# marlbenchmark/off-policy

Hardware: NVIDIA H100
Metric: learner grad-steps/sec (higher is better)
Workload: dtype f32

## Files before the change

### off-policy_b200/csrc/agent_bwd.cu

```cuda
#include "mx_internal.h"
#include "mx_kernels.h"
#include "mx_tile.cuh"
#include "mx_mma.cuh"

static inline size_t qhead_bwd_smem(int A) { return (size_t)(A * MX_H * 9 + 8 * 32 + 2 * 8 * MX_H + 2 * MX_H) * sizeof(float); }

__global__ void __launch_bounds__(256) k_qhead_bwd(QHeadBwdArgs a) {
  MX_DYN_SMEM(smem);
  const int tid = threadIdx.x, lane = tid & 31, warp = tid >> 5;
  const int A = a.A, AW = A * MX_H;
  float* wq_s = smem;
  float* dw_w = wq_s + AW;
  float* db_w = dw_w + 8 * AW;
  float* dg_w = db_w + 8 * 32;
  float* dbt_w = dg_w + 8 * MX_H;
  float* lg_s = dbt_w + 8 * MX_H;
  float* lb_s = lg_s + MX_H;
  for (int i = tid; i < AW; i += blockDim.x) wq_s[i] = a.theta[a.wq + i];
  for (int i = tid; i < 8 * AW + 8 * 32; i += blockDim.x) dw_w[i] = 0.f;
  for (int i = tid; i < MX_H; i += blockDim.x) { lg_s[i] = a.theta[a.lno_g + i]; lb_s[i] = a.theta[a.lno_b + i]; }
  MX_PDL_WAIT();
  __syncthreads();
  const int wglobal = blockIdx.x * (blockDim.x >> 5) + warp;
  const int wtotal = gridDim.x * (blockDim.x >> 5);
// ... 247 lines not shown
        if (rok[r]) mx_cp16z(pf_dst + ((t & (RING - 1)) * ROWS + r) * (6 * MX_H), first ? (pf_h0[r] ? pf_h0[r] : a.hall) : pf_src[r], (first && !pf_h0[r]) ? 0 : 16);
        pf_src[r] -= pf_stride;
      }
    }
    mx_cp_commit();
  };
  if (ROWS > 1) {
    for (int idx = tid; idx < RING * ROWS * 6 * MX_H; idx += BWD2_THREADS) (&ops_s[0][0][0][0])[idx] = 0.f;
    __syncthreads();
  }
#pragma unroll
  for (int d = 0; d < PF; ++d) prefetch(t_first - d);
  mx_cp_wait<PF - 1>();
  __syncthreads();

  auto step = [&](const int t, const int cur) {
    prefetch(t - PF);
    float cz[ROWS];
#pragma unroll
    for (int r = 0; r < ROWS; ++r) {
      const float* o = &ops_s[t & (RING - 1)][r][0][0];
      const float rg = o[ku], zg = o[MX_H + ku], ng = o[2 * MX_H + ku], hn = o[3 * MX_H + ku], hp = o[4 * MX_H + ku];
      const float dh = o[5 * MX_H + ku] + carry[r];
      const float d_n = dh * (1.f - zg) * (1.f - ng * ng);
      const float d_z = dh * (hp - ng) * zg * (1.f - zg);
      const float d_r = d_n * hn * rg * (1.f - rg);
      dgh_s[cur][r][(half ? 2 * MX_H : 0) + ku] = half ? d_n * rg : d_r;
      if (!half) dgh_s[cur][r][MX_H + ku] = d_z;
      if (rok[r]) {
        dgp[r][half ? 2 * MX_H : 0] = half ? d_n : d_r;
        if (!half) dgp[r][MX_H] = d_z;
      }
      dgp[r] -= dg_stride;
      cz[r] = dh * zg;
    }
    mx_cp_wait<PF - 1>();
    __syncthreads();
#pragma unroll
    for (int r = 0; r < ROWS; ++r) {
      float2 a0 = make_float2(0.f, 0.f), a1 = a0, b0 = a0, b1 = a0;
#pragma unroll
      for (int m = 0; m < 12; ++m) {
        const float4 d = mx_ld4(&dgh_s[cur][r][16 * m + 4 * s]);
        const float2 lo = make_float2(d.x, d.y), hi = make_float2(d.z, d.w);
        a0 = mx_ffma2(w0[2 * m], lo, a0); b0 = mx_ffma2(w1[2 * m], lo, b0);
        a1 = mx_ffma2(w0[2 * m + 1], hi, a1); b1 = mx_ffma2(w1[2 * m + 1], hi, b1);
      }
      a0 = mx_fadd2(a0, a1); b0 = mx_fadd2(b0, b1);
      float p0 = a0.x + a0.y, p1 = b0.x + b0.y;
      p0 += __shfl_xor_sync(0xffffffffu, p0, 1); p1 += __shfl_xor_sync(0xffffffffu, p1, 1);
      p0 += __shfl_xor_sync(0xffffffffu, p0, 2); p1 += __shfl_xor_sync(0xffffffffu, p1, 2);
      carry[r] = cz[r] + ((s & 1) ? p1 : p0);
    }
  };
  int t = t_first;
  for (; t >= 1; t -= 2) { step(t, 0); step(t - 1, 1); }
  if (t == 0) step(0, 0);
  mx_cp_wait<0>();
}

struct FrontBwdSmem {
  int ldi, ld64, ldg;
  int o_dgi, o_dgn, o_x, o_hp, o_u, o_da, o_x0, o_xh0, o_dx0, o_wc, o_col, o_stat, o_lnp, total;
};
static FrontBwdSmem front_bwd_smem(int in_dim, int TM, bool gru_ext = false) {
  FrontBwdSmem s;
  const int I64 = mx_round_up(in_dim, 64);
  s.ldi = mx_ld(I64); s.ld64 = mx_ld(64); s.ldg = mx_ld(MX_G);
  int o = 0;
  s.o_dgi = o; o += TM * s.ldg;
  s.o_dgn = o; o += gru_ext ? 0 : TM * s.ld64;
  s.o_x = o; o += TM * s.ld64;
  s.o_hp = o; o += gru_ext ? 0 : TM * s.ld64;
  s.o_u = o; o += TM * s.ld64;
  s.o_da = o; o += TM * s.ld64;
  s.o_x0 = o; o += TM * s.ldi;
  s.o_xh0 = o; o += TM * s.ldi;
  s.o_dx0 = o; o += TM * s.ldi;
  s.o_wc = o; o += 64 * s.ld64;
  s.o_col = o; o += 2 * I64 + 4 * 64;
  s.o_stat = o; o += 3 * TM * 2;
  s.o_lnp = o; o += 4 * 64;
  s.total = o;
  return s;
}

template <int RM>
MX_DEVINL void ln64_bwd_relu(bool act_tanh, float (&v)[RM][4], const float* u_s, int ld, const float* stat , const float* gamma_s,
                             float (&dg)[4], float (&db)[4]) {
  const int tx = threadIdx.x & 15, ty = threadIdx.x >> 4;
#pragma unroll
  for (int i = 0; i < RM; ++i) {
    const int r = ty * RM + i;
    const float mean = stat[2 * r], rstd = stat[2 * r + 1];
    const float4 u4 = mx_ld4(u_s + r * ld + 4 * tx);
    const float uu[4] = {u4.x, u4.y, u4.z, u4.w};
    float xh[4], dx[4], s1 = 0.f, s2 = 0.f;
#pragma unroll
    for (int j = 0; j < 4; ++j) {
      xh[j] = (uu[j] - mean) * rstd;
      dg[j] = fmaf(v[i][j], xh[j], dg[j]);
      db[j] += v[i][j];
      dx[j] = v[i][j] * gamma_s[4 * tx + j];
      s1 += dx[j]; s2 += dx[j] * xh[j];
    }
    s1 = mx_row16_sum(s1) * (1.f / 64.f);
    s2 = mx_row16_sum(s2) * (1.f / 64.f);
#pragma unroll
    for (int j = 0; j < 4; ++j) {
      const float du = rstd * (dx[j] - s1 - xh[j] * s2);
      v[i][j] = act_tanh ? du * (1.f - uu[j] * uu[j]) : (uu[j] > 0.f ? du : 0.f);
    }
  }
}

template <int RM, bool MMA>
__global__ void __launch_bounds__(MX_TILE_THREADS) k_front_bwd(FrontBwdArgs a, FrontBwdSmem sm) {
  constexpr int TM = 16 * RM;
  MX_DYN_SMEM(smem);
  const MxNetLayout L = a.L;
  const float* __restrict__ th = a.theta;
  const int I = L.in_dim, I64 = mx_round_up(I, 64);
  float* dgi_s = smem + sm.o_dgi; float* dgn_s = smem + sm.o_dgn; float* x_s = smem + sm.o_x; float* hp_s = smem + sm.o_hp;
  float* u_s = smem + sm.o_u; float* da_s = smem + sm.o_da; float* x0_s = smem + sm.o_x0; float* xh0_s = smem + sm.o_xh0;
  float* Wc = smem + sm.o_wc;
  float* col0g = smem + sm.o_col; float* col0b = col0g + I64;
  float* col1g = col0b + I64; float* col1b = col1g + 64;
  float* col2g = col1b + 64; float* col2b = col2g + 64;
  float* st0_s = smem + sm.o_stat; float* st1_s = st0_s + 2 * TM; float* st2_s = st1_s + 2 * TM;
  float* ln1g_s = smem + sm.o_lnp; float* ln1b_s = ln1g_s + 64; float* ln2g_s = ln1b_s + 64; float* ln2b_s = ln2g_s + 64;
  const int tid = threadIdx.x, tx = tid & 15, ty = tid >> 4;
  const int ntiles = (a.M + TM - 1) / TM;
  const int T1 = a.T1 > 0 ? a.T1 : a.T + 1, N = a.N;
  const bool ldx_vec = (a.ldx & 3) == 0;
  const bool wg = !a.skip_wgrad;
  const bool wgemm = wg && !a.wgrad_external;
  const bool gru_here = !a.gru_wgrad_ext;
  float* dx0_s = smem + sm.o_dx0;
  float* gp = a.gpart + (size_t)blockIdx.x * a.P;
  for (int i = tid; i < 2 * I64 + 4 * 64; i += MX_TILE_THREADS) col0g[i] = 0.f;
  if (tid < 64) { ln1g_s[tid] = th[L.ln1_g + tid]; ln1b_s[tid] = th[L.ln1_b + tid]; ln2g_s[tid] = th[L.ln2_g + tid]; ln2b_s[tid] = th[L.ln2_b + tid]; }
  float dg1[4] = {0.f, 0.f, 0.f, 0.f}, db1[4] = {0.f, 0.f, 0.f, 0.f}, dg2[4] = {0.f, 0.f, 0.f, 0.f}, db2[4] = {0.f, 0.f, 0.f, 0.f};
  int iter = 0;
  MX_PDL_WAIT();
  for (int tile = blockIdx.x; tile < ntiles; tile += gridDim.x, ++iter) {
    const int m0 = tile * TM;
    const bool accum = iter > 0;
    __syncthreads();
    mx_stage_rows(dgi_s, sm.ldg, a.dgi, MX_G, m0, a.M, TM, MX_G);
    if (!gru_here) {}
    else if (!a.no_gru) mx_stage_rows(x_s, sm.ld64, a.gates, MX_G, m0, a.M, TM, MX_H);
    else for (int i = tid; i < TM * sm.ld64; i += MX_TILE_THREADS) x_s[i] = 0.f;
    mx_stage_rows(u_s, sm.ld64, a.u2, MX_H, m0, a.M, TM, MX_H);
    for (int r = tid >> 4; gru_here && r < TM; r += MX_TILE_THREADS / 16) {
      const int m = m0 + r;
      const bool has = !a.no_gru && m < a.M && ((m / N) % T1) > 0;
      float* d = hp_s + r * sm.ld64 + 4 * tx;
      if (has) mx_cp16(d, a.hall + (size_t)(m - N) * MX_H + 4 * tx);
      else if (m < a.M && a.h0) mx_cp16(d, a.h0 + (size_t)m * MX_H + 4 * tx);
      else mx_st4(d, make_float4(0.f, 0.f, 0.f, 0.f));
    }
    if (ldx_vec) mx_stage_rows(x0_s, sm.ldi, a.X, a.ldx, m0, a.M, TM, mx_round_up(I, 4));
    mx_cp_commit();
    for (int i = tid; i < 3 * TM * 2; i += MX_TILE_THREADS) {
      const int which = i / (2 * TM), rr = (i % (2 * TM)) >> 1, comp = i & 1;
      const int m = m0 + rr;
      const float* src = which == 0 ? a.st0 : (which == 1 ? a.st1 : a.st2);
      st0_s[i] = (m < a.M && (which > 0 || a.feature_norm)) ? src[2 * (size_t)m + comp] : 0.f;
    }
    mx_cp_wait<0>();
    __syncthreads();
    for (int idx = tid; gru_here && idx < TM * MX_H; idx += MX_TILE_THREADS) {
      const int r = idx >> 6, c = idx & 63;
      const int o = r * sm.ld64 + c;
      dgn_s[o] = dgi_s[r * sm.ldg + 2 * MX_H + c] * x_s[o];
      x_s[o] = (m0 + r < a.M) ? (u_s[o] - st2_s[2 * r]) * st2_s[2 * r + 1] * ln2g_s[c] + ln2b_s[c] : 0.f;
    }
    __syncthreads();
    if (wgemm && gru_here) {
      for (int nb = 0; nb < 3; ++nb) {
        if (MMA) mx_mma_wgrad_block(dgi_s + nb * 64, sm.ldg, x_s, sm.ld64, TM, gp + L.wih, MX_G, MX_H, nb * 64, 0, accum);
        else mx_wgrad_block(dgi_s + nb * 64, sm.ldg, x_s, sm.ld64, TM, gp + L.wih, MX_G, MX_H, nb * 64, 0, accum);
        if (a.no_gru) continue;
        const float* dgh = nb < 2 ? dgi_s + nb * 64 : dgn_s;
        const int ldd = nb < 2 ? sm.ldg : sm.ld64;
        if (MMA) mx_mma_wgrad_block(dgh, ldd, hp_s, sm.ld64, TM, gp + L.whh + nb * 64 * MX_H, 64, MX_H, 0, 0, accum);
        else mx_wgrad_block(dgh, ldd, hp_s, sm.ld64, TM, gp + L.whh + nb * 64 * MX_H, 64, MX_H, 0, 0, accum);
      }
      mx_colsum(dgi_s, sm.ldg, TM, MX_G, gp + L.bih, accum);
      if (!a.no_gru) {
        mx_colsum(dgi_s, sm.ldg, TM, 2 * MX_H, gp + L.bhh, accum);
        mx_colsum(dgn_s, sm.ld64, TM, MX_H, gp + L.bhh + 2 * MX_H, accum);
      }
    }
    float v[RM][4];
#pragma unroll
    for (int i = 0; i < RM; ++i)
#pragma unroll
      for (int jx = 0; jx < 4; ++jx) v[i][jx] = 0.f;
    if (MMA) {
      float cfr[RM][4];
#pragma unroll
      for (int i = 0; i < RM; ++i)
#pragma unroll
        for (int jx = 0; jx < 4; ++jx) cfr[i][jx] = 0.f;
      for (int nc = 0; nc < 3; ++nc) {
        __syncthreads();
        mx_stage_weight(Wc, sm.ld64, th + L.wih, MX_G, MX_H, MX_H, nc * 64, 0, 64);
        __syncthreads();
        mx_mma_dgrad_acc<RM>(cfr, dgi_s + nc * 64, sm.ldg, Wc, sm.ld64);
      }
      mx_mma_store<RM>(cfr, da_s, sm.ld64);
      __syncthreads();
#pragma unroll
      for (int i = 0; i < RM; ++i) {
        const float4 q = mx_ld4(da_s + (ty * RM + i) * sm.ld64 + 4 * tx);
        v[i][0] = q.x; v[i][1] = q.y; v[i][2] = q.z; v[i][3] = q.w;
      }
    } else
    for (int nc = 0; nc < 3; ++nc) {
      __syncthreads();
      mx_stage_weight(Wc, sm.ld64, th + L.wih, MX_G, MX_H, MX_H, nc * 64, 0, 64);
      __syncthreads();
      mx_mm_nn<RM>(dgi_s + nc * 64, sm.ldg, Wc, sm.ld64, v);
    }
    ln64_bwd_relu<RM>(a.act_tanh != 0, v, u_s, sm.ld64, st2_s, ln2g_s, dg2, db2);
    __syncthreads();
#pragma unroll
    for (int i = 0; i < RM; ++i) mx_st4(da_s + (ty * RM + i) * sm.ld64 + 4 * tx, make_float4(v[i][0], v[i][1], v[i][2], v[i][3]));
    if (a.wgrad_external) {
#pragma unroll
      for (int i = 0; i < RM; ++i) {
        const int m = m0 + ty * RM + i;
        if (m < a.M) mx_st4(a.da2_out + (size_t)m * MX_H + 4 * tx, make_float4(v[i][0], v[i][1], v[i][2], v[i][3]));
      }
    }
    mx_stage_rows(u_s, sm.ld64, a.u1, MX_H, m0, a.M, TM, MX_H);
    mx_cp_commit();
    mx_cp_wait<0>();
    __syncthreads();
    for (int idx = tid; idx < TM * MX_H; idx += MX_TILE_THREADS) {
      const int r = idx >> 6, c = idx & 63;
      const int o = r * sm.ld64 + c;
      x_s[o] = (m0 + r < a.M) ? (u_s[o] - st1_s[2 * r]) * st1_s[2 * r + 1] * ln1g_s[c] + ln1b_s[c] : 0.f;
    }
    __syncthreads();
    if (wgemm) {
      if (MMA) mx_mma_wgrad_block(da_s, sm.ld64, x_s, sm.ld64, TM, gp + L.w2, MX_H, MX_H, 0, 0, accum);
      else mx_wgrad_block(da_s, sm.ld64, x_s, sm.ld64, TM, gp + L.w2, MX_H, MX_H, 0, 0, accum);
      mx_colsum(da_s, sm.ld64, TM, MX_H, gp + L.b2, accum);
    }
    mx_stage_weight(Wc, sm.ld64, th + L.w2, MX_H, MX_H, MX_H, 0, 0, 64);
    __syncthreads();
#pragma unroll
    for (int i = 0; i < RM; ++i)
#pragma unroll
      for (int jx = 0; jx < 4; ++jx) v[i][jx] = 0.f;
    if (MMA) {
      float cfr[RM][4];
#pragma unroll
      for (int i = 0; i < RM; ++i)
#pragma unroll
        for (int jx = 0; jx < 4; ++jx) cfr[i][jx] = 0.f;
      mx_mma_dgrad_acc<RM>(cfr, da_s, sm.ld64, Wc, sm.ld64);
      mx_mma_store<RM>(cfr, x_s, sm.ld64);
      __syncthreads();
#pragma unroll
      for (int i = 0; i < RM; ++i) {
        const float4 q = mx_ld4(x_s + (ty * RM + i) * sm.ld64 + 4 * tx);
        v[i][0] = q.x; v[i][1] = q.y; v[i][2] = q.z; v[i][3] = q.w;
      }
    } else
    mx_mm_nn<RM>(da_s, sm.ld64, Wc, sm.ld64, v);
    ln64_bwd_relu<RM>(a.act_tanh != 0, v, u_s, sm.ld64, st1_s, ln1g_s, dg1, db1);
    __syncthreads();
#pragma unroll
    for (int i = 0; i < RM; ++i) mx_st4(da_s + (ty * RM + i) * sm.ld64 + 4 * tx, make_float4(v[i][0], v[i][1], v[i][2], v[i][3]));
    if (a.wgrad_external) {
#pragma unroll
      for (int i = 0; i < RM; ++i) {
        const int m = m0 + ty * RM + i;
        if (m < a.M) mx_st4(a.da1_out + (size_t)m * MX_H + 4 * tx, make_float4(v[i][0], v[i][1], v[i][2], v[i][3]));
      }
    }
    for (int idx = tid; idx < TM * I64; idx += MX_TILE_THREADS) {
      const int r = idx / I64, c = idx - r * I64, m = m0 + r;
      float xh = 0.f, x0 = 0.f;
      if (m < a.M && c < I) {
        const float x = ldx_vec ? x0_s[r * sm.ldi + c] : a.X[(size_t)m * a.ldx + c];
        if (a.feature_norm) {
          xh = (x - st0_s[2 * r]) * st0_s[2 * r + 1];
          x0 = xh * th[L.fn_g + c] + th[L.fn_b + c];
        } else x0 = x;
      }
      x0_s[r * sm.ldi + c] = x0; xh0_s[r * sm.ldi + c] = xh;
    }
    __syncthreads();
    if (wgemm) {
      for (int kb = 0; kb * 64 < I; ++kb) {
        if (MMA) mx_mma_wgrad_block(da_s, sm.ld64, x0_s + kb * 64, sm.ldi, TM, gp + L.w1, MX_H, I, 0, kb * 64, accum);
        else mx_wgrad_block(da_s, sm.ld64, x0_s + kb * 64, sm.ldi, TM, gp + L.w1, MX_H, I, 0, kb * 64, accum);
      }
      mx_colsum(da_s, sm.ld64, TM, MX_H, gp + L.b1, accum);
    }
    if (a.feature_norm || a.dX) {
      for (int kb = 0; kb * 64 < I; ++kb) {
        __syncthreads();
        mx_stage_weight(Wc, sm.ld64, th + L.w1, MX_H, I, I, 0, kb * 64, 64);
        __syncthreads();
#pragma unroll
        for (int i = 0; i < RM; ++i)
#pragma unroll
          for (int jx = 0; jx < 4; ++jx) v[i][jx] = 0.f;
        if (MMA) {
          float cfr[RM][4];
#pragma unroll
          for (int i = 0; i < RM; ++i)
#pragma unroll
            for (int jx = 0; jx < 4; ++jx) cfr[i][jx] = 0.f;
          mx_mma_dgrad_acc<RM>(cfr, da_s, sm.ld64, Wc, sm.ld64);
          mx_mma_store<RM>(cfr, dx0_s + kb * 64, sm.ldi);
          __syncthreads();
#pragma unroll
          for (int i = 0; i < RM; ++i) {
            const float4 q = mx_ld4(dx0_s + (ty * RM + i) * sm.ldi + kb * 64 + 4 * tx);
            v[i][0] = q.x; v[i][1] = q.y; v[i][2] = q.z; v[i][3] = q.w;
          }
        } else
        mx_mm_nn<RM>(da_s, sm.ld64, Wc, sm.ld64, v);
        float cg[4] = {0.f, 0.f, 0.f, 0.f}, cb[4] = {0.f, 0.f, 0.f, 0.f};
#pragma unroll
        for (int jx = 0; jx < 4; ++jx) {
          const int c = kb * 64 + 4 * tx + jx;
          if (c < I) {
            float sg = 0.f, sb = 0.f;
#pragma unroll
            for (int i = 0; i < RM; ++i) {
              sg = fmaf(v[i][jx], xh0_s[(ty * RM + i) * sm.ldi + c], sg); sb += v[i][jx];
              if (a.dX) dx0_s[(ty * RM + i) * sm.ldi + c] = v[i][jx];
            }
            cg[jx] = sg; cb[jx] = sb;
          }
        }
        if (wg && a.feature_norm) {
          for (int g = 0; g < MX_TILE_THREADS / 16; ++g) {
            if (ty == g) {
#pragma unroll
              for (int jx = 0; jx < 4; ++jx) {
                const int c = kb * 64 + 4 * tx + jx;
                if (c < I) { col0g[c] += cg[jx]; col0b[c] += cb[jx]; }
              }
            }
            __syncthreads();
          }
        }
      }
      if (a.dX) {
        __syncthreads();
        const int lane = tid & 31, warp = tid >> 5;
        for (int r = warp; r < TM; r += MX_TILE_THREADS / 32) {
          const int m = m0 + r;
          if (m >= a.M) continue;
          float s1 = 0.f, s2 = 0.f;
          for (int c = lane; c < I; c += 32) {
            const float dxh = dx0_s[r * sm.ldi + c] * (a.feature_norm ? th[L.fn_g + c] : 1.f);
            s1 += dxh; s2 += dxh * xh0_s[r * sm.ldi + c];
          }
          s1 = mx_warp_sum(s1) / (float)I; s2 = mx_warp_sum(s2) / (float)I;
          const float rstd = st0_s[2 * r + 1];
          for (int c = lane; c < I; c += 32) {
            const float d0 = dx0_s[r * sm.ldi + c];
            a.dX[(size_t)m * a.ldx + c] = a.feature_norm ? rstd * (d0 * th[L.fn_g + c] - s1 - xh0_s[r * sm.ldi + c] * s2) : d0;
          }
        }
      }
    }
  }
  for (int g = 0; g < MX_TILE_THREADS / 16; ++g) {
    if (ty == g) {
#pragma unroll
      for (int jx = 0; jx < 4; ++jx) {
        const int c = 4 * tx + jx;
        col1g[c] += dg1[jx]; col1b[c] += db1[jx];
        col2g[c] += dg2[jx]; col2b[c] += db2[jx];
      }
    }
    __syncthreads();
  }
  if (wg) {
    for (int c = tid; c < MX_H; c += MX_TILE_THREADS) {
      gp[L.ln2_g + c] = col2g[c]; gp[L.ln2_b + c] = col2b[c];
      gp[L.ln1_g + c] = col1g[c]; gp[L.ln1_b + c] = col1b[c];
    }
    for (int c = tid; c < I; c += MX_TILE_THREADS) { gp[L.fn_g + c] = col0g[c]; gp[L.fn_b + c] = col0b[c]; }
  }
}


struct GruWgradSmem { int ld64, ldg, o_dgi, o_dgn, o_x, o_hp, o_stat, o_lnp, total; };
static GruWgradSmem gru_wgrad_smem(int TM) {
  GruWgradSmem s;
  s.ld64 = mx_ld(64); s.ldg = mx_ld(MX_G);
  int o = 0;
  s.o_dgi = o; o += TM * s.ldg;
  s.o_dgn = o; o += TM * s.ld64;
  s.o_x = o; o += TM * s.ld64;
  s.o_hp = o; o += TM * s.ld64;
  s.o_stat = o; o += 2 * TM;
  s.o_lnp = o; o += 2 * 64;
  s.total = o;
  return s;
}

template <int RM>
__global__ void __launch_bounds__(MX_TILE_THREADS, 2) k_gru_wgrad(FrontBwdArgs a, GruWgradSmem sm) {
  constexpr int TM = 16 * RM;
  MX_DYN_SMEM(smem);
  const MxNetLayout L = a.L;
  const float* __restrict__ th = a.theta;
  float* dgi_s = smem + sm.o_dgi; float* dgn_s = smem + sm.o_dgn; float* x_s = smem + sm.o_x; float* hp_s = smem + sm.o_hp;
  float* st2_s = smem + sm.o_stat; float* ln2g_s = smem + sm.o_lnp; float* ln2b_s = ln2g_s + 64;
  const int tid = threadIdx.x, tx = tid & 15;
  const int tk = tid & 7, tn = tid >> 3;
  const int ntiles = (a.M + TM - 1) / TM;
  const int T1 = a.T1 > 0 ? a.T1 : a.T + 1, N = a.N;
  float* gp = a.gpart + (size_t)blockIdx.x * a.P;
  if (tid < 64) { ln2g_s[tid] = th[L.ln2_g + tid]; ln2b_s[tid] = th[L.ln2_b + tid]; }
  int iter = 0;
  MX_PDL_WAIT();
  for (int tile = blockIdx.x; tile < ntiles; tile += gridDim.x, ++iter) {
    const int m0 = tile * TM;
    __syncthreads();
    mx_stage_rows(dgi_s, sm.ldg, a.dgi, MX_G, m0, a.M, TM, MX_G);
    mx_stage_rows(dgn_s, sm.ld64, a.gates, MX_G, m0, a.M, TM, MX_H);
    mx_stage_rows(x_s, sm.ld64, a.u2, MX_H, m0, a.M, TM, MX_H);
    for (int r = tid >> 4; r < TM; r += MX_TILE_THREADS / 16) {
      const int m = m0 + r;
      const bool has = m < a.M && ((m / N) % T1) > 0;
// ... 68 lines not shown
  const int cap = mx_num_sms();
  if (grid > cap) grid = cap;
  if (grid < 1) grid = 1;
  const size_t smem = qhead_bwd_smem(a.A);
#if !MX_EMU
  static size_t configured = 0;
  if (smem > 48 * 1024 && smem > configured) {
    if (cudaFuncSetAttribute(k_qhead_bwd, cudaFuncAttributeMaxDynamicSharedMemorySize, (int)smem) != cudaSuccess) { mx_set_error("qhead_bwd: smem %zu too large", smem); return 1; }
    configured = smem;
  }
#endif
  MX_LAUNCH_PDL(k_qhead_bwd, dim3(grid), dim3(256), smem, s, a);
  MX_COUNT();
  MX_MARK("k_qhead_bwd", s);
  *nparts_used = grid;
  return MX_CHECK_LAUNCH("qhead_bwd");
}

__global__ void __launch_bounds__(256) k_mlp_dgi(const float* __restrict__ dq_taken, const int32_t* __restrict__ act_idx, int ld_tn,
                                                 float* __restrict__ dgi, int B, int N) {
  const long long total = (long long)B * 2 * N * MX_G;
  MX_PDL_WAIT();
  for (long long i = (long long)blockIdx.x * blockDim.x + threadIdx.x; i < total; i += (long long)gridDim.x * blockDim.x) {
    const int c = (int)(i % MX_G);
    const long long m = i / MX_G;
    const int n = (int)(m % N);
    const long long bt = m / N;
    const int t = (int)(bt & 1);
    const long long b = bt >> 1;
    float v = 0.f;
    if (t == 0 && c == act_idx[b * ld_tn + n]) v = dq_taken[b * N + n];
    dgi[i] = v;
  }
}
int mx_launch_mlp_dgi(const float* dq_taken, const int32_t* act_idx, int ld_tn, float* dgi, int B, int N, cudaStream_t s) {
  const long long total = (long long)B * 2 * N * MX_G;
  int grid = (int)((total + 255) / 256);
  const int cap = mx_num_sms() * 8;
  if (grid > cap) grid = cap;
  MX_LAUNCH_PDL(k_mlp_dgi, dim3(grid), dim3(256), 0, s, dq_taken, act_idx, ld_tn, dgi, B, N);
  MX_COUNT();
  MX_MARK("k_mlp_dgi", s);
  return MX_CHECK_LAUNCH("mlp_dgi");
}

int mx_launch_gru_bwd(const GruBwdArgs& a, cudaStream_t s) {
  const int sms = mx_num_sms();
  int rpc = 1;
  while (rpc < 4 && mx_ceil_div(a.R, rpc) > 2 * sms) rpc *= 2;
  if (g_mx_gru_bwd_rpc == 1 || g_mx_gru_bwd_rpc == 2 || g_mx_gru_bwd_rpc == 4) rpc = g_mx_gru_bwd_rpc;
  if (g_mx_gru_threads == 128 || (g_mx_gru_threads == 0 && g_mx_gru_bwd_rpc == 0 && a.T >= 8)) {
    const bool two = g_mx_gru_rows == 2 || (g_mx_gru_rows == 0 && a.R > 2 * mx_num_sms());
    if (two) MX_LAUNCH_PDL(k_gru_bwd2<2>, dim3((a.R + 1) / 2), dim3(BWD2_THREADS), 0, s, a);
    else MX_LAUNCH_PDL(k_gru_bwd2<1>, dim3(a.R), dim3(BWD2_THREADS), 0, s, a);
    MX_COUNT();
    MX_MARK("k_gru_bwd", s);
    return MX_CHECK_LAUNCH("gru_bwd2");
  }
  dim3 grid(mx_ceil_div(a.R, rpc));
  if (rpc == 1) MX_LAUNCH_PDL(k_gru_bwd<1>, grid, dim3(BWD_THREADS), 0, s, a);
  else if (rpc == 2) MX_LAUNCH_PDL(k_gru_bwd<2>, grid, dim3(BWD_THREADS), 0, s, a);
  else MX_LAUNCH_PDL(k_gru_bwd<4>, grid, dim3(BWD_THREADS), 0, s, a);
  MX_COUNT();
  MX_MARK("k_gru_bwd", s);
  return MX_CHECK_LAUNCH("gru_bwd");
}

static int front_bwd_pick_rm(int M, int in_dim, int sms, bool gru_ext) {
  int best = 2;
  double best_cost = 1e30;
  for (int rm = 2; rm <= 4; ++rm) {
    FrontBwdSmem sm = front_bwd_smem(in_dim, 16 * rm, gru_ext);
    if ((size_t)sm.total * sizeof(float) + 16 > 227 * 1024) continue;
    const int tiles = mx_ceil_div(M, 16 * rm);
    const double cost = (double)mx_ceil_div(tiles, sms) * (1.0 + rm);
    if (cost < best_cost - 1e-9) { best_cost = cost; best = rm; }
  }
  return best;
}

template <int RM, bool MMA>
static int front_bwd_launch(const FrontBwdArgs& a, int* nparts_used, cudaStream_t s) {
  const int TM = 16 * RM;
  FrontBwdSmem sm = front_bwd_smem(a.L.in_dim, TM, a.gru_wgrad_ext != 0);
  const size_t smem = (size_t)sm.total * sizeof(float) + 16;
  const int ntiles = mx_ceil_div(a.M, TM);
  int grid = mx_num_sms();
  if (grid > ntiles) grid = ntiles;
  auto kern = k_front_bwd<RM, MMA>;
#if !MX_EMU
  if (smem > 227 * 1024) { mx_set_error("front_bwd: %zu bytes of shared memory needed (obs_dim too large)", smem); return 1; }
  static size_t configured = 0;
  if (smem > configured) { cudaFuncSetAttribute(kern, cudaFuncAttributeMaxDynamicSharedMemorySize, (int)smem); configured = smem; }
#endif
  MX_LAUNCH_PDL(kern, dim3(grid), dim3(MX_TILE_THREADS), smem, s, a, sm);
  MX_COUNT();
  MX_MARK("k_front_bwd", s);
  *nparts_used = grid;
  return MX_CHECK_LAUNCH("front_bwd");
}

extern int g_mx_front_bwd_rm;
int g_mx_gru_wgrad_split = 1;
int g_mx_front_bwd_mma = 0;
bool mx_front_bwd_tc_usable(const FrontBwdArgs& a);
int mx_launch_front_bwd_tc(const FrontBwdArgs& a, int* nparts_used, cudaStream_t s);
// ... 47 lines not shown
```

### off-policy_b200/csrc/agent_fwd.cu

```cuda
#include "mx_internal.h"
#include "mx_kernels.h"
#include "mx_tile.cuh"

template <int RM>
__global__ void __launch_bounds__(MX_TILE_THREADS) k_front_fwd(FrontFwdArgs a) {
  constexpr int TM = 16 * RM;
  MX_DYN_SMEM(smem);
  const int net = blockIdx.y;
  const float* __restrict__ th = a.theta[net];
  const MxNetLayout L = a.L;
  const int I = L.in_dim, Ipad = (I + 3) & ~3;
  const int lda = mx_ld_dev(Ipad > MX_H ? Ipad : MX_H);
  const int ldw = lda;
  float* A_s = smem;
  float* Wc = A_s + TM * lda;
  const int tid = threadIdx.x, tx = tid & 15, ty = tid >> 4, lane = tid & 31, warp = tid >> 5;
  const bool live = (net == 0);
  const int ntiles = (a.M + TM - 1) / TM;
  MX_PDL_WAIT();

  for (int tile = blockIdx.x; tile < ntiles; tile += gridDim.x) {
    const int m0 = tile * TM;
    if (I <= 128) {
      constexpr int RW = TM / (MX_TILE_THREADS / 32);
// ... 265 lines not shown
  const bool on1 = q == 0 || live, on2 = live, on3 = live && q == 0;
  const size_t s1 = (size_t)N * ((q == 0) ? MX_H : MX_G), s2 = (size_t)N * MX_G, s3 = (size_t)N * MX_H;
  float* pf_dst = &gi_s[0][0][4 * (pf_on ? tid : 0)];
  const size_t pf_stride = (size_t)N * MX_G;
  auto prefetch = [&](int t) {
    if (pf_on && t < T1) {
#pragma unroll
      for (int r = 0; r < ROWS; ++r) {
        if (rok[r]) mx_cp16(pf_dst + ((t & (GRU_RING - 1)) * ROWS + r) * MX_G, pf_src[r]);
        pf_src[r] += pf_stride;
      }
    }
    mx_cp_commit();
  };
#pragma unroll
  for (int t = 0; t < GRU_PF; ++t) prefetch(t);
  mx_cp_wait<GRU_PF - 1>();
  __syncthreads();

  auto step = [&](const int t, const int cur) {
    const int nxt = cur ^ 1;
    prefetch(t + GRU_PF);
#pragma unroll
    for (int r = 0; r < ROWS; ++r) {
      const float* g = &gi_s[t & (GRU_RING - 1)][r][0];
      const float* hrow = &h_s[cur][r][0];
      float4 hv[8];
#pragma unroll
      for (int m = 0; m < 8; ++m) hv[m] = mx_ld4(hrow + 8 * m + 4 * q);
      const float gr = g[i] + br, gz = g[MX_H + i] + bz, gn = g[2 * MX_H + i], hp = hrow[i];
      float2 r0 = make_float2(0.f, 0.f), r1 = r0, z0 = r0, z1 = r0, n0 = r0, n1 = r0;
#pragma unroll
      for (int m = 0; m < 8; ++m) {
        const float2 lo = make_float2(hv[m].x, hv[m].y), hi = make_float2(hv[m].z, hv[m].w);
        r0 = mx_ffma2(wr[2 * m], lo, r0); n0 = mx_ffma2(wn[2 * m], lo, n0); z0 = mx_ffma2(wz[2 * m], lo, z0);
        r1 = mx_ffma2(wr[2 * m + 1], hi, r1); n1 = mx_ffma2(wn[2 * m + 1], hi, n1); z1 = mx_ffma2(wz[2 * m + 1], hi, z1);
      }
      r0 = mx_fadd2(r0, r1); n0 = mx_fadd2(n0, n1); z0 = mx_fadd2(z0, z1);
      float pr = r0.x + r0.y, pn = n0.x + n0.y, pz = z0.x + z0.y;
      pr += __shfl_xor_sync(0xffffffffu, pr, 1); pn += __shfl_xor_sync(0xffffffffu, pn, 1); pz += __shfl_xor_sync(0xffffffffu, pz, 1);
      const float rg = mx_sigmoid_fast(pr + gr);
      const float hn = pn + bn;
      const float ng = mx_tanh_fast(fmaf(rg, hn, gn));
      const float zg = mx_sigmoid_fast(pz + gz);
      const float hnew = fmaf(zg, hp - ng, ng);
      h_s[nxt][r][i] = hnew;
      if (rok[r]) {
        if (on1) *p1[r] = q == 0 ? hnew : zg;
        if (on2) *p2[r] = q == 0 ? rg : ng;
        if (on3) *p3[r] = hn;
      }
      p1[r] += s1; p2[r] += s2; p3[r] += s3;
    }
    mx_cp_wait<GRU_PF - 1>();
    __syncthreads();
  };
  int t = 0;
  for (; t + 1 < T1; t += 2) { step(t, 0); step(t + 1, 1); }
  if (t < T1) step(t, 0);
  mx_cp_wait<0>();
}

__global__ void __launch_bounds__(256) k_qhead(QHeadArgs a) {
  __shared__ float wq_s[2][32 * MX_H];
  __shared__ float bq_s[2][32];
  __shared__ float lg_s[2][MX_H], lb_s[2][MX_H];
  const int tid = threadIdx.x, lane = tid & 31;
  const int A = a.A;
  for (int net = 0; net < 2; ++net) {
    const float* th = a.theta[net];
    for (int i = tid; i < A * MX_H; i += blockDim.x) wq_s[net][i] = th[a.wq + i];
    for (int i = tid; i < A; i += blockDim.x) bq_s[net][i] = th[a.bq + i];
    for (int i = tid; i < MX_H; i += blockDim.x) { lg_s[net][i] = th[a.lno_g + i]; lb_s[net][i] = th[a.lno_b + i]; }
  }
  MX_PDL_WAIT();
  __syncthreads();
  const int wglobal = blockIdx.x * (blockDim.x >> 5) + (tid >> 5);
  const int wtotal = gridDim.x * (blockDim.x >> 5);
  const int T1 = a.T + 1, N = a.N;
  for (int m = wglobal; m < a.M; m += wtotal) {
    const int n = m % N;
    const int bt = m / N;
    const int t = bt % T1, b = bt / T1;
    float q_live_at_act = 0.f, tq_sel = 0.f;
    int greedy = 0;
    const float* hl = a.hall[0] + (size_t)m * MX_H;
    const float* ht = a.hall[1] + (size_t)m * MX_H;
    const float hl0 = hl[lane], hl1 = hl[lane + 32], ht0 = ht[lane], ht1 = ht[lane + 32];
    const int act = (t < a.T) ? a.act_idx[(size_t)b * a.ld_tn + (size_t)t * N + n] : 0;
    float av = 1.f;
    if (a.avail && lane < A) av = a.avail[(size_t)m * a.act_ld + lane];
    const unsigned avail_mask = __ballot_sync(0xffffffffu, av != 0.f);
    {
      const float mean = mx_warp_sum(hl0 + hl1) * (1.f / MX_H);
      const float d0 = hl0 - mean, d1 = hl1 - mean;
      const float rstd = rsqrtf(mx_warp_sum(d0 * d0 + d1 * d1) * (1.f / MX_H) + MX_LN_EPS);
      if (lane == 0) { a.sto[2 * (size_t)m] = mean; a.sto[2 * (size_t)m + 1] = rstd; }
      const float y0 = d0 * rstd * lg_s[0][lane] + lb_s[0][lane];
      const float y1 = d1 * rstd * lg_s[0][lane + 32] + lb_s[0][lane + 32];
      float best = 0.f;
      for (int k = 0; k < A; ++k) {
        float q = mx_warp_sum(y0 * wq_s[0][k * MX_H + lane] + y1 * wq_s[0][k * MX_H + lane + 32]) + bq_s[0][k];
        if (a.qall0 && lane == 0) a.qall0[(size_t)m * A + k] = q;
        if (k == act) q_live_at_act = q;
        const float qm = ((avail_mask >> k) & 1u) ? q : -1e10f;
        if (k == 0 || qm > best) { best = qm; greedy = k; }
// ... 79 lines not shown

int mx_launch_pack_prev_act(const float* obs, int obs_ld, const float* acts, int act_ld, float* X, int ldx, int B, int T, int N, int O, int A,
                            cudaStream_t s) {
  const long long total = (long long)B * (T + 1) * N * ldx;
  int grid = (int)((total + 255) / 256);
  const int cap = mx_num_sms() * 8;
  if (grid > cap) grid = cap;
  MX_LAUNCH_PDL(k_pack_prev_act, dim3(grid), dim3(256), 0, s, obs, obs_ld, acts, act_ld, X, ldx, B, T, N, O, A);
  MX_COUNT();
  MX_MARK("k_pack_prev_act", s);
  return MX_CHECK_LAUNCH("pack_prev_act");
}

size_t mx_front_fwd_smem(int in_dim, int RM) {
  const int Ipad = mx_round_up(in_dim, 4);
  const int lda = mx_ld(Ipad > MX_H ? Ipad : MX_H);
  return (size_t)(16 * RM + 64) * lda * sizeof(float);
}

extern int g_mx_front_tc;
int mx_launch_front_fwd_tc(const FrontFwdArgs& a, int nets, cudaStream_t s);
bool mx_front_tc_usable(int in_dim, bool have_image);

int mx_launch_front_fwd(const FrontFwdArgs& a, int nets, cudaStream_t s) {
  if (mx_front_tc_usable(a.L.in_dim, a.tc_img[0] != nullptr) && (a.ldx & 3) == 0) return mx_launch_front_fwd_tc(a, nets, s);
  const int RM = 2;
  const int ntiles = mx_ceil_div(a.M, 16 * RM);
  int gx = mx_num_sms() / nets;
  if (gx < 1) gx = 1;
  if (gx > ntiles) gx = ntiles;
  const size_t smem = mx_front_fwd_smem(a.L.in_dim, RM);
  auto kern = k_front_fwd<2>;
#if !MX_EMU
  static size_t configured = 0;
  if (smem > configured) {
    if (cudaFuncSetAttribute(kern, cudaFuncAttributeMaxDynamicSharedMemorySize, (int)smem) != cudaSuccess) { mx_set_error("front_fwd: smem %zu too large", smem); return 1; }
    configured = smem;
  }
#endif
  MX_LAUNCH_PDL(kern, dim3(gx, nets), dim3(MX_TILE_THREADS), smem, s, a);
  MX_COUNT();
  MX_MARK("k_front_fwd", s);
  return MX_CHECK_LAUNCH("front_fwd");
}

int mx_launch_gru_fwd(const GruFwdArgs& a, int nets, cudaStream_t s) {
  const int sms = mx_num_sms();
  int rpc = 1;
  while (rpc < 4 && mx_ceil_div(a.R, rpc) * nets > 2 * sms) rpc *= 2;
  if (g_mx_gru_fwd_rpc == 1 || g_mx_gru_fwd_rpc == 2 || g_mx_gru_fwd_rpc == 4) rpc = g_mx_gru_fwd_rpc;
  if (g_mx_gru_threads == 128 || (g_mx_gru_threads == 0 && g_mx_gru_fwd_rpc == 0 && a.T + 1 >= 8)) {
    const bool two = g_mx_gru_rows == 2 || (g_mx_gru_rows == 0 && (long long)a.R * nets > 2LL * mx_num_sms());
    if (two) MX_LAUNCH_PDL(k_gru_fwd2<2>, dim3((a.R + 1) / 2, nets), dim3(GRU2_THREADS), 0, s, a);
    else MX_LAUNCH_PDL(k_gru_fwd2<1>, dim3(a.R, nets), dim3(GRU2_THREADS), 0, s, a);
    MX_COUNT();
    MX_MARK("k_gru_fwd", s);
    return MX_CHECK_LAUNCH("gru_fwd2");
  }
  dim3 grid(mx_ceil_div(a.R, rpc), nets);
  if (rpc == 1) MX_LAUNCH_PDL(k_gru_fwd<1>, grid, dim3(GRU_THREADS), 0, s, a);
  else if (rpc == 2) MX_LAUNCH_PDL(k_gru_fwd<2>, grid, dim3(GRU_THREADS), 0, s, a);
  else MX_LAUNCH_PDL(k_gru_fwd<4>, grid, dim3(GRU_THREADS), 0, s, a);
  MX_COUNT();
  MX_MARK("k_gru_fwd", s);
  return MX_CHECK_LAUNCH("gru_fwd");
}

int mx_launch_qhead(const QHeadArgs& a, cudaStream_t s) {
  if (a.A > 32) { mx_set_error("qhead: act_dim %d > 32 unsupported", a.A); return 1; }
  int grid = mx_ceil_div(a.M, 8);
  const int cap = mx_num_sms() * 4;
  if (grid > cap) grid = cap;
  MX_LAUNCH_PDL(k_qhead, dim3(grid), dim3(256), 0, s, a);
  MX_COUNT();
  MX_MARK("k_qhead", s);
  return MX_CHECK_LAUNCH("qhead");
}
```

Baseline: 4731.

## Prefetch MLP weight chunks asynchronously and parallelize LN column reductions

Issues asynchronous cp.async staging of the first weight chunk for each dgrad GEMM (wih, w2, w1) earlier, so the copies overlap with the preceding elementwise work and the barriers around them drop away. It also replaces the serialized per-row-group accumulation loops (one __syncthreads per group) for the feature-norm and layernorm gamma/beta gradients with a shared-memory partial buffer followed by a parallel column reduction. The cost is reuse of dgi_s as scratch and more fragile ordering of async copies and barriers.

```diff
diff --git a/off-policy_b200/csrc/agent_bwd.cu b/off-policy_b200/csrc/agent_bwd.cu
--- a/off-policy_b200/csrc/agent_bwd.cu
+++ b/off-policy_b200/csrc/agent_bwd.cu
@@ -413,11 +413,13 @@
   if (tid < 64) { ln1g_s[tid] = th[L.ln1_g + tid]; ln1b_s[tid] = th[L.ln1_b + tid]; ln2g_s[tid] = th[L.ln2_g + tid]; ln2b_s[tid] = th[L.ln2_b + tid]; }
   float dg1[4] = {0.f, 0.f, 0.f, 0.f}, db1[4] = {0.f, 0.f, 0.f, 0.f}, dg2[4] = {0.f, 0.f, 0.f, 0.f}, db2[4] = {0.f, 0.f, 0.f, 0.f};
   int iter = 0;
+  mx_stage_weight(Wc, sm.ld64, th + L.wih, MX_G, MX_H, MX_H, 0, 0, 64, false);
   MX_PDL_WAIT();
   for (int tile = blockIdx.x; tile < ntiles; tile += gridDim.x, ++iter) {
     const int m0 = tile * TM;
     const bool accum = iter > 0;
     __syncthreads();
+    if (iter > 0) mx_stage_weight(Wc, sm.ld64, th + L.wih, MX_G, MX_H, MX_H, 0, 0, 64, false);
     mx_stage_rows(dgi_s, sm.ldg, a.dgi, MX_G, m0, a.M, TM, MX_G);
     if (!gru_here) {}
     else if (!a.no_gru) mx_stage_rows(x_s, sm.ld64, a.gates, MX_G, m0, a.M, TM, MX_H);
@@ -476,27 +478,32 @@
 #pragma unroll
         for (int jx = 0; jx < 4; ++jx) cfr[i][jx] = 0.f;
       for (int nc = 0; nc < 3; ++nc) {
+        if (nc > 0) {
+          __syncthreads();
+          mx_stage_weight(Wc, sm.ld64, th + L.wih, MX_G, MX_H, MX_H, nc * 64, 0, 64);
+          __syncthreads();
+        }
+        mx_mma_dgrad_acc<RM>(cfr, dgi_s + nc * 64, sm.ldg, Wc, sm.ld64);
+      }
+      mx_mma_store<RM>(cfr, da_s, sm.ld64);
+      __syncthreads();
+#pragma unroll
+      for (int i = 0; i < RM; ++i) {
+        const float4 q = mx_ld4(da_s + (ty * RM + i) * sm.ld64 + 4 * tx);
+        v[i][0] = q.x; v[i][1] = q.y; v[i][2] = q.z; v[i][3] = q.w;
+      }
+    } else
+    for (int nc = 0; nc < 3; ++nc) {
+      if (nc > 0) {
         __syncthreads();
         mx_stage_weight(Wc, sm.ld64, th + L.wih, MX_G, MX_H, MX_H, nc * 64, 0, 64);
         __syncthreads();
-        mx_mma_dgrad_acc<RM>(cfr, dgi_s + nc * 64, sm.ldg, Wc, sm.ld64);
-      }
-      mx_mma_store<RM>(cfr, da_s, sm.ld64);
-      __syncthreads();
-#pragma unroll
-      for (int i = 0; i < RM; ++i) {
-        const float4 q = mx_ld4(da_s + (ty * RM + i) * sm.ld64 + 4 * tx);
-        v[i][0] = q.x; v[i][1] = q.y; v[i][2] = q.z; v[i][3] = q.w;
-      }
-    } else
-    for (int nc = 0; nc < 3; ++nc) {
-      __syncthreads();
-      mx_stage_weight(Wc, sm.ld64, th + L.wih, MX_G, MX_H, MX_H, nc * 64, 0, 64);
-      __syncthreads();
+      }
       mx_mm_nn<RM>(dgi_s + nc * 64, sm.ldg, Wc, sm.ld64, v);
     }
     ln64_bwd_relu<RM>(a.act_tanh != 0, v, u_s, sm.ld64, st2_s, ln2g_s, dg2, db2);
     __syncthreads();
+    mx_stage_weight(Wc, sm.ld64, th + L.w2, MX_H, MX_H, MX_H, 0, 0, 64, false);
 #pragma unroll
     for (int i = 0; i < RM; ++i) mx_st4(da_s + (ty * RM + i) * sm.ld64 + 4 * tx, make_float4(v[i][0], v[i][1], v[i][2], v[i][3]));
     if (a.wgrad_external) {
@@ -521,7 +528,6 @@
       else mx_wgrad_block(da_s, sm.ld64, x_s, sm.ld64, TM, gp + L.w2, MX_H, MX_H, 0, 0, accum);
       mx_colsum(da_s, sm.ld64, TM, MX_H, gp + L.b2, accum);
     }
-    mx_stage_weight(Wc, sm.ld64, th + L.w2, MX_H, MX_H, MX_H, 0, 0, 64);
     __syncthreads();
 #pragma unroll
     for (int i = 0; i < RM; ++i)
@@ -545,6 +551,8 @@
     mx_mm_nn<RM>(da_s, sm.ld64, Wc, sm.ld64, v);
     ln64_bwd_relu<RM>(a.act_tanh != 0, v, u_s, sm.ld64, st1_s, ln1g_s, dg1, db1);
     __syncthreads();
+    const bool dx0_wanted = a.feature_norm || a.dX;
+    if (dx0_wanted) mx_stage_weight(Wc, sm.ld64, th + L.w1, MX_H, I, I, 0, 0, 64, false);
 #pragma unroll
     for (int i = 0; i < RM; ++i) mx_st4(da_s + (ty * RM + i) * sm.ld64 + 4 * tx, make_float4(v[i][0], v[i][1], v[i][2], v[i][3]));
     if (a.wgrad_external) {
@@ -574,10 +582,11 @@
       }
       mx_colsum(da_s, sm.ld64, TM, MX_H, gp + L.b1, accum);
     }
-    if (a.feature_norm || a.dX) {
+    if (dx0_wanted) {
       for (int kb = 0; kb * 64 < I; ++kb) {
         __syncthreads();
-        mx_stage_weight(Wc, sm.ld64, th + L.w1, MX_H, I, I, 0, kb * 64, 64);
+        if (kb > 0) mx_stage_weight(Wc, sm.ld64, th + L.w1, MX_H, I, I, 0, kb * 64, 64);
+        else mx_cp_wait<0>();
         __syncthreads();
 #pragma unroll
         for (int i = 0; i < RM; ++i)
@@ -614,16 +623,23 @@
           }
         }
         if (wg && a.feature_norm) {
-          for (int g = 0; g < MX_TILE_THREADS / 16; ++g) {
-            if (ty == g) {
-#pragma unroll
-              for (int jx = 0; jx < 4; ++jx) {
-                const int c = kb * 64 + 4 * tx + jx;
-                if (c < I) { col0g[c] += cg[jx]; col0b[c] += cb[jx]; }
-              }
+          float* part = dgi_s;
+#pragma unroll
+          for (int jx = 0; jx < 4; ++jx) {
+            part[(2 * ty) * 64 + 4 * tx + jx] = cg[jx];
+            part[(2 * ty + 1) * 64 + 4 * tx + jx] = cb[jx];
+          }
+          __syncthreads();
+          if (tid < 128) {
+            const int which = tid >> 6, c = kb * 64 + (tid & 63);
+            if (c < I) {
+              float* col = which ? col0b : col0g;
+              float s = col[c];
+              for (int g = 0; g < MX_TILE_THREADS / 16; ++g) s += part[(2 * g + which) * 64 + (tid & 63)];
+              col[c] = s;
             }
-            __syncthreads();
           }
+          __syncthreads();
         }
       }
       if (a.dX) {
@@ -647,14 +663,21 @@
       }
     }
   }
-  for (int g = 0; g < MX_TILE_THREADS / 16; ++g) {
-    if (ty == g) {
-#pragma unroll
-      for (int jx = 0; jx < 4; ++jx) {
-        const int c = 4 * tx + jx;
-        col1g[c] += dg1[jx]; col1b[c] += db1[jx];
-        col2g[c] += dg2[jx]; col2b[c] += db2[jx];
-      }
+  {
+    float* part = dgi_s;
+#pragma unroll
+    for (int jx = 0; jx < 4; ++jx) {
+      const int c = 4 * tx + jx;
+      part[(4 * ty) * 64 + c] = dg1[jx]; part[(4 * ty + 1) * 64 + c] = db1[jx];
+      part[(4 * ty + 2) * 64 + c] = dg2[jx]; part[(4 * ty + 3) * 64 + c] = db2[jx];
+    }
+    __syncthreads();
+    {
+      const int which = tid >> 6, c = tid & 63;
+      float* col = which == 0 ? col1g : which == 1 ? col1b : which == 2 ? col2g : col2b;
+      float s = col[c];
+      for (int g = 0; g < MX_TILE_THREADS / 16; ++g) s += part[(4 * g + which) * 64 + c];
+      col[c] = s;
     }
     __syncthreads();
   }
```

Result: faster. 4789 (median of 6 runs) (+1.2%).

## Add repartitioned single-row GRU forward and backward recurrence kernels

Applied to the files above, without the earlier changes.

Adds new k_gru_fwd3 and k_gru_bwd3 kernels for the one-row-per-block case. They split the hidden-state matvec across threads differently: each thread keeps a wider set of recurrent weights in float2 registers and partial sums are combined with fewer xor shuffles. The backward kernel also prefetches all six per-step operands into a shared-memory ring with cp.async. The aim is to shorten the serial per-timestep latency of the recurrence, at the cost of higher register pressure (launch bounds of 2 blocks per SM) and more code paths. They run only when the default thread setting picks the single-row path.

```diff
diff --git a/off-policy_b200/csrc/agent_bwd.cu b/off-policy_b200/csrc/agent_bwd.cu
--- a/off-policy_b200/csrc/agent_bwd.cu
+++ b/off-policy_b200/csrc/agent_bwd.cu
@@ -323,6 +323,99 @@
       p0 += __shfl_xor_sync(0xffffffffu, p0, 2); p1 += __shfl_xor_sync(0xffffffffu, p1, 2);
       carry[r] = cz[r] + ((s & 1) ? p1 : p0);
     }
+  };
+  int t = t_first;
+  for (; t >= 1; t -= 2) { step(t, 0); step(t - 1, 1); }
+  if (t == 0) step(0, 0);
+  mx_cp_wait<0>();
+}
+
+__global__ void __launch_bounds__(BWD2_THREADS, 2) k_gru_bwd3(GruBwdArgs a) {
+  constexpr int RING = 8, PF = 6;
+  __shared__ __align__(16) float ops_s[RING][6][MX_H];
+  __shared__ __align__(16) float dgh_s[2][MX_G];
+  const int tid = threadIdx.x;
+  const int c4 = tid >> 3, s = (tid >> 1) & 3, cp = tid & 1, half = s >> 1;
+  const int ku = 4 * c4 + 2 * cp + (s & 1);
+  float2 w[4][12];
+#pragma unroll
+  for (int m = 0; m < 12; ++m) {
+    const float* wp = a.theta + a.whh + (16 * m + 4 * s + 2 * cp) * MX_H + 4 * c4;
+#pragma unroll
+    for (int cc = 0; cc < 4; ++cc) w[cc][m] = make_float2(wp[cc], wp[MX_H + cc]);
+  }
+  const int T1 = a.T1 > 0 ? a.T1 : a.T + 1, N = a.N;
+  MX_PDL_WAIT();
+  const int t_first = a.T - 1;
+  const bool pf_on = tid < 96;
+  const int op = pf_on ? tid / 16 : 0, q4 = tid % 16;
+  const bool pf_hprev = op == 4;
+  const size_t pf_stride = (size_t)N * (op < 3 ? MX_G : MX_H);
+  const size_t dg_stride = (size_t)N * MX_G;
+  const int row = blockIdx.x;
+  const bool rok = row < a.R;
+  const int rr = rok ? row : 0;
+  const size_t m0 = ((size_t)(rr / N) * T1) * N + (rr % N);
+  const float* base = op < 3 ? a.gates + m0 * MX_G + op * MX_H + 4 * q4 : (op == 3 ? a.hn : (op == 4 ? a.hall : a.dh_out)) + m0 * MX_H + 4 * q4;
+  const float* pf_src = base + (ptrdiff_t)(pf_hprev ? t_first - 1 : t_first) * (ptrdiff_t)pf_stride;
+  const float* pf_h0 = (pf_hprev && a.h0) ? a.h0 + (size_t)rr * MX_H + 4 * q4 : nullptr;
+  if (rok)
+    for (int tz = a.T; tz < T1; ++tz)
+      for (int c = tid; c < MX_G; c += BWD2_THREADS) a.dgi[(m0 + (size_t)tz * N) * MX_G + c] = 0.f;
+  float* dgp = a.dgi + (m0 + (size_t)t_first * N) * MX_G + ku;
+  float carry = 0.f;
+  float* pf_dst = &ops_s[0][op][4 * q4];
+  auto prefetch = [&](int t) {
+    if (t >= 0 && pf_on && rok) {
+      const bool first = pf_hprev && t == 0;
+      mx_cp16z(pf_dst + (t & (RING - 1)) * (6 * MX_H), first ? (pf_h0 ? pf_h0 : a.hall) : pf_src, (first && !pf_h0) ? 0 : 16);
+      pf_src -= pf_stride;
+    }
+    mx_cp_commit();
+  };
+#pragma unroll
+  for (int d = 0; d < PF; ++d) prefetch(t_first - d);
+  mx_cp_wait<PF - 1>();
+  __syncthreads();
+
+  auto step = [&](const int t, const int cur) {
+    prefetch(t - PF);
+    const float* o = &ops_s[t & (RING - 1)][0][0];
+    const float rg = o[ku], zg = o[MX_H + ku], ng = o[2 * MX_H + ku], hn = o[3 * MX_H + ku], hp = o[4 * MX_H + ku];
+    const float dh = o[5 * MX_H + ku] + carry;
+    const float d_n = dh * (1.f - zg) * (1.f - ng * ng);
+    const float d_z = dh * (hp - ng) * zg * (1.f - zg);
+    const float d_r = d_n * hn * rg * (1.f - rg);
+    dgh_s[cur][(half ? 2 * MX_H : 0) + ku] = half ? d_n * rg : d_r;
+    if (!half) dgh_s[cur][MX_H + ku] = d_z;
+    if (rok) {
+      dgp[half ? 2 * MX_H : 0] = half ? d_n : d_r;
+      if (!half) dgp[MX_H] = d_z;
+    }
+    dgp -= dg_stride;
+    const float cz = dh * zg;
+    mx_cp_wait<PF - 1>();
+    __syncthreads();
+    float2 acc[4];
+#pragma unroll
+    for (int cc = 0; cc < 4; ++cc) acc[cc] = make_float2(0.f, 0.f);
+#pragma unroll
+    for (int m = 0; m < 12; ++m) {
+      const float2 d = *reinterpret_cast<const float2*>(&dgh_s[cur][16 * m + 4 * s + 2 * cp]);
+#pragma unroll
+      for (int cc = 0; cc < 4; ++cc) acc[cc] = mx_ffma2(w[cc][m], d, acc[cc]);
+    }
+    float sv[2];
+#pragma unroll
+    for (int e = 0; e < 2; ++e) {
+      const float2 keep = cp ? acc[2 + e] : acc[e], give = cp ? acc[e] : acc[2 + e];
+      const float ox = __shfl_xor_sync(0xffffffffu, give.x, 1), oy = __shfl_xor_sync(0xffffffffu, give.y, 1);
+      sv[e] = (keep.x + ox) + (keep.y + oy);
+    }
+    float kk = (s & 1) ? sv[1] : sv[0];
+    kk += __shfl_xor_sync(0xffffffffu, (s & 1) ? sv[0] : sv[1], 2);
+    kk += __shfl_xor_sync(0xffffffffu, kk, 4);
+    carry = cz + kk;
   };
   int t = t_first;
   for (; t >= 1; t -= 2) { step(t, 0); step(t - 1, 1); }
@@ -829,6 +922,7 @@
   if (g_mx_gru_threads == 128 || (g_mx_gru_threads == 0 && g_mx_gru_bwd_rpc == 0 && a.T >= 8)) {
     const bool two = g_mx_gru_rows == 2 || (g_mx_gru_rows == 0 && a.R > 2 * mx_num_sms());
     if (two) MX_LAUNCH_PDL(k_gru_bwd2<2>, dim3((a.R + 1) / 2), dim3(BWD2_THREADS), 0, s, a);
+    else if (g_mx_gru_threads == 0) MX_LAUNCH_PDL(k_gru_bwd3, dim3(a.R), dim3(BWD2_THREADS), 0, s, a);
     else MX_LAUNCH_PDL(k_gru_bwd2<1>, dim3(a.R), dim3(BWD2_THREADS), 0, s, a);
     MX_COUNT();
     MX_MARK("k_gru_bwd", s);
diff --git a/off-policy_b200/csrc/agent_fwd.cu b/off-policy_b200/csrc/agent_fwd.cu
--- a/off-policy_b200/csrc/agent_fwd.cu
+++ b/off-policy_b200/csrc/agent_fwd.cu
@@ -341,6 +341,103 @@
       }
       p1[r] += s1; p2[r] += s2; p3[r] += s3;
     }
+    mx_cp_wait<GRU_PF - 1>();
+    __syncthreads();
+  };
+  int t = 0;
+  for (; t + 1 < T1; t += 2) { step(t, 0); step(t + 1, 1); }
+  if (t < T1) step(t, 0);
+  mx_cp_wait<0>();
+}
+
+__global__ void __launch_bounds__(GRU2_THREADS, 2) k_gru_fwd3(GruFwdArgs a) {
+  __shared__ __align__(16) float h_s[2][MX_H];
+  __shared__ __align__(16) float gi_s[GRU_RING][MX_G];
+  const int net = blockIdx.y;
+  const float* __restrict__ th = net ? a.theta[1] : a.theta[0];
+  const int tid = threadIdx.x;
+  const int p = tid >> 2, half = (tid >> 1) & 1, cp = tid & 1;
+  const int u = 2 * p + cp;
+  const bool live = (net == 0) && a.gates != nullptr;
+  float2 w[3][2][8];
+#pragma unroll
+  for (int g = 0; g < 3; ++g)
+#pragma unroll
+    for (int e = 0; e < 2; ++e)
+#pragma unroll
+      for (int m = 0; m < 8; ++m) {
+        const float* wp = th + a.whh + (g * MX_H + 2 * p + e) * MX_H + 8 * m + 4 * half + 2 * cp;
+        w[g][e][m] = make_float2(wp[0], wp[1]);
+      }
+  const float br = th[a.bhh + u], bz = th[a.bhh + MX_H + u], bn = th[a.bhh + 2 * MX_H + u];
+  MX_PDL_WAIT();
+  const float* gi = net ? a.gi[1] : a.gi[0];
+  float* hall = net ? a.hall[1] : a.hall[0];
+  const int T1 = a.T + 1, N = a.N;
+  const int row = blockIdx.x;
+  const bool rok = row < a.R;
+  const int rr = rok ? row : 0;
+  if (tid < 2 * MX_H) (&h_s[0][0])[tid] = (a.h0 && tid < MX_H && rok) ? a.h0[(size_t)rr * MX_H + tid] : 0.f;
+  const size_t m0 = ((size_t)(rr / N) * T1) * N + (rr % N);
+  float* p1 = half == 0 ? hall + m0 * MX_H + u : (live ? a.gates + m0 * MX_G + MX_H + u : hall);
+  float* p2 = live ? a.gates + m0 * MX_G + (half == 0 ? 0 : 2 * MX_H) + u : hall;
+  float* p3 = live ? a.hn + m0 * MX_H + u : hall;
+  const bool on1 = rok && (half == 0 || live), on2 = rok && live, on3 = rok && live && half == 0;
+  const size_t s1 = (size_t)N * ((half == 0) ? MX_H : MX_G), s2 = (size_t)N * MX_G, s3 = (size_t)N * MX_H;
+  const bool pf_on = tid < MX_G / 4 && rok;
+  const float* pf_src = gi + m0 * MX_G + 4 * (pf_on ? tid : 0);
+  float* pf_dst = &gi_s[0][4 * (pf_on ? tid : 0)];
+  const size_t pf_stride = (size_t)N * MX_G;
+  auto prefetch = [&](int t) {
+    if (pf_on && t < T1) { mx_cp16(pf_dst + (t & (GRU_RING - 1)) * MX_G, pf_src); pf_src += pf_stride; }
+    mx_cp_commit();
+  };
+#pragma unroll
+  for (int t = 0; t < GRU_PF; ++t) prefetch(t);
+  mx_cp_wait<GRU_PF - 1>();
+  __syncthreads();
+
+  auto step = [&](const int t, const int cur) {
+    const int nxt = cur ^ 1;
+    prefetch(t + GRU_PF);
+    const float* g = &gi_s[t & (GRU_RING - 1)][0];
+    const float* hrow = &h_s[cur][0];
+    float2 hv[8];
+#pragma unroll
+    for (int m = 0; m < 8; ++m) hv[m] = *reinterpret_cast<const float2*>(hrow + 8 * m + 4 * half + 2 * cp);
+    const float gr = g[u] + br, gz = g[MX_H + u] + bz, gn = g[2 * MX_H + u], hp = hrow[u];
+    float2 acc[3][2];
+#pragma unroll
+    for (int gg = 0; gg < 3; ++gg)
+#pragma unroll
+      for (int e = 0; e < 2; ++e) acc[gg][e] = make_float2(0.f, 0.f);
+#pragma unroll
+    for (int m = 0; m < 8; ++m)
+#pragma unroll
+      for (int gg = 0; gg < 3; ++gg) {
+        const int gr_ = gg == 0 ? 0 : (gg == 1 ? 2 : 1);
+#pragma unroll
+        for (int e = 0; e < 2; ++e) acc[gr_][e] = mx_ffma2(w[gr_][e][m], hv[m], acc[gr_][e]);
+      }
+    float pre[3];
+#pragma unroll
+    for (int gg = 0; gg < 3; ++gg) {
+      const float2 keep = cp ? acc[gg][1] : acc[gg][0], give = cp ? acc[gg][0] : acc[gg][1];
+      const float ox = __shfl_xor_sync(0xffffffffu, give.x, 1), oy = __shfl_xor_sync(0xffffffffu, give.y, 1);
+      pre[gg] = (keep.x + ox) + (keep.y + oy);
+    }
+    float pr = pre[0], pz = pre[1], pn = pre[2];
+    pr += __shfl_xor_sync(0xffffffffu, pr, 2); pn += __shfl_xor_sync(0xffffffffu, pn, 2); pz += __shfl_xor_sync(0xffffffffu, pz, 2);
+    const float rg = mx_sigmoid_fast(pr + gr);
+    const float hn = pn + bn;
+    const float ng = mx_tanh_fast(fmaf(rg, hn, gn));
+    const float zg = mx_sigmoid_fast(pz + gz);
+    const float hnew = fmaf(zg, hp - ng, ng);
+    h_s[nxt][u] = hnew;
+    if (on1) *p1 = half == 0 ? hnew : zg;
+    if (on2) *p2 = half == 0 ? rg : ng;
+    if (on3) *p3 = hn;
+    p1 += s1; p2 += s2; p3 += s3;
     mx_cp_wait<GRU_PF - 1>();
     __syncthreads();
   };
@@ -526,6 +623,7 @@
   if (g_mx_gru_threads == 128 || (g_mx_gru_threads == 0 && g_mx_gru_fwd_rpc == 0 && a.T + 1 >= 8)) {
     const bool two = g_mx_gru_rows == 2 || (g_mx_gru_rows == 0 && (long long)a.R * nets > 2LL * mx_num_sms());
     if (two) MX_LAUNCH_PDL(k_gru_fwd2<2>, dim3((a.R + 1) / 2, nets), dim3(GRU2_THREADS), 0, s, a);
+    else if (g_mx_gru_threads == 0) MX_LAUNCH_PDL(k_gru_fwd3, dim3(a.R, nets), dim3(GRU2_THREADS), 0, s, a);
     else MX_LAUNCH_PDL(k_gru_fwd2<1>, dim3(a.R, nets), dim3(GRU2_THREADS), 0, s, a);
     MX_COUNT();
     MX_MARK("k_gru_fwd", s);
```

After: 4692 before, 4955 after (median of 6 runs). 1.06x the previous value.
